# castorini/howl

Hardware: AMD Instinct MI355X
Metric: utterances/sec/node (res8 end-to-end training step, 1s@16kHz, 40-mel) (higher is better)
Workload: dtype f32; 1 GPU; res8 training step (frontend+fwd+xent+bwd+AdamW), 512 x 1 s utterances per GPU, 12 labels -- BASELINE configs[2] per-GPU share: res8 GSC-12, 512 x 1 s per GPU (4096 over 8); global_batch=512, samples_per_utterance=16000, labels=12, parallelism=single, frontend=eval

## Files before the change

howl_amd/csrc/howl_common.hip.h:

```cpp
#pragma once
#include <hip/hip_runtime.h>
#include <math.h>
#include <stdint.h>
#include <stdio.h>

typedef float f32x4 __attribute__((ext_vector_type(4)));
typedef __attribute__((address_space(3))) float lds_f32;

#if defined(HIPEMU)
#define HOWL_OPAQUE_V(x) ((void)(x))
#else
#define HOWL_OPAQUE_V(x) asm volatile("" : "+v"(x))
#endif
#define HOWL_OPAQUE_LDS(p) HOWL_OPAQUE_V(p)
#if defined(HIPEMU)
#define HOWL_SCHED_PIN() ((void)0)
#else
#define HOWL_SCHED_PIN() __builtin_amdgcn_sched_barrier(0)
#endif

#define HOWL_OK 0
#define HOWL_E_ARG (-1)
#define HOWL_E_LAUNCH (-2)
#define HOWL_E_WORKSPACE (-3)

void howl_set_error(const char* fmt, ...);
int howl_num_cus();
bool howl_prof_begin(const char* tag, hipStream_t stream, size_t* slot, double work);
void howl_prof_end(size_t slot, hipStream_t stream);

struct HowlSideLane {
    hipStream_t stream;
    hipEvent_t fork_ev, join_ev;
};
HowlSideLane* howl_side_lane();
bool howl_raise_lds(const void* kernel, size_t lds, size_t* granted, const char* what);
bool howl_take_pending_error();
inline void howl_lane_fork(HowlSideLane* l, hipStream_t main) {
    hipEventRecord(l->fork_ev, main);
    hipStreamWaitEvent(l->stream, l->fork_ev, 0);
}
inline void howl_lane_join(HowlSideLane* l, hipStream_t main) {
    hipEventRecord(l->join_ev, l->stream);
    hipStreamWaitEvent(main, l->join_ev, 0);
}

struct HowlProfScope {
    size_t slot = 0;
    bool on;
    hipStream_t stream;
    HowlProfScope(const char* tag, hipStream_t s, double work = 0.0) : stream(s) { on = howl_prof_begin(tag, s, &slot, work); }
    ~HowlProfScope() {
        if (on) howl_prof_end(slot, stream);
    }
};

struct HowlAdamWCoef {
    float lr, b1, b2, eps, wd, bc1, bc2_sqrt, gscale;
};
inline HowlAdamWCoef howl_adamw_coef(float lr, float beta1, float beta2, float eps, float weight_decay, int step, float grad_scale) {
    const double bc1 = 1.0 - pow((double)beta1, (double)step);
    const double bc2 = 1.0 - pow((double)beta2, (double)step);
    return HowlAdamWCoef{lr, beta1, beta2, eps, weight_decay, (float)bc1, (float)sqrt(bc2), grad_scale};
}
__device__ __forceinline__ void howl_adamw_element(float* __restrict__ p, float* __restrict__ m, float* __restrict__ v, size_t i, float g,
                                                   const HowlAdamWCoef& c) {
#pragma clang fp contract(off)
    const float gi = g * c.gscale;
    float pi = p[i] * (1.0f - c.lr * c.wd);
    const float mi = m[i] + (gi - m[i]) * (1.0f - c.b1);
    const float vi = c.b2 * v[i] + (1.0f - c.b2) * gi * gi;
    const float denom = sqrtf(vi) / c.bc2_sqrt + c.eps;
    pi -= (c.lr / c.bc1) * (mi / denom);
    p[i] = pi;
    m[i] = mi;
    v[i] = vi;
}

#define HOWL_REQUIRE(cond, ...)                 \
    do {                                        \
        if (!(cond)) {                          \
            howl_set_error(__VA_ARGS__);        \
            return HOWL_E_ARG;                  \
        }                                       \
    } while (0)

#define HOWL_CHECK_LAUNCH(name)                                                     \
    do {                                                                            \
        hipError_t e_ = hipGetLastError();                                          \
        if (howl_take_pending_error()) return HOWL_E_LAUNCH;   \
        if (e_ != hipSuccess) {                                                     \
            howl_set_error("%s: launch failed: %s", name, hipGetErrorString(e_));   \
            return HOWL_E_LAUNCH;                                                   \
        }                                                                           \
    } while (0)

__device__ __forceinline__ void wave_lds_sync() {
    __builtin_amdgcn_fence(__ATOMIC_RELEASE, "wavefront");
    __builtin_amdgcn_wave_barrier();
    __builtin_amdgcn_fence(__ATOMIC_ACQUIRE, "wavefront");
}

__device__ __forceinline__ float wave_sum(float v) {
    for (int m = 32; m >= 1; m >>= 1) v += __shfl_xor(v, m);
    return v;
}
__device__ __forceinline__ float wave_sum_rows(float v) {
    v += __int_as_float(__builtin_amdgcn_update_dpp(0, __float_as_int(v), 0xB1, 0xf, 0xf, true));
    v += __int_as_float(__builtin_amdgcn_update_dpp(0, __float_as_int(v), 0x4E, 0xf, 0xf, true));
    v += __int_as_float(__builtin_amdgcn_update_dpp(0, __float_as_int(v), 0x141, 0xf, 0xf, true));
    v += __int_as_float(__builtin_amdgcn_update_dpp(0, __float_as_int(v), 0x140, 0xf, 0xf, true));
    v += __shfl_xor(v, 16);
    v += __shfl_xor(v, 32);
    return v;
}
__device__ __forceinline__ double wave_sum_d(double v) {
    for (int m = 32; m >= 1; m >>= 1) v += __shfl_xor(v, m);
    return v;
}
```

howl_amd/csrc/res8.hip:

```cpp
#include "howl_common.hip.h"
#include "../../include/howl_hip.h"

namespace {

struct HowlPtrs6 {
    float* p[6];
};
constexpr int MAX_WINDOWS = 64;
struct HowlWinRows {
    int lo[MAX_WINDOWS], hi[MAX_WINDOWS];
};
struct HowlBnBuffers {
    float* running_mean;
    float* running_var;
    long long* num_batches;
};
struct BnFold {
    const float* part;
    int nparts;
    double count;
    float* stats_out;
    HowlBnBuffers bn;
};


constexpr int NMAP = 45;
constexpr int CP = 48;
constexpr int PW = 10;
constexpr int WP = 12;
constexpr int CONV_THREADS = 768;
constexpr int KFULL = 11;
constexpr int KSTEPS = 9 * KFULL + 3;
constexpr int MAX_H = 27;
constexpr int MAX_ROW_STRIPS = 1024;
constexpr float BN_EPS = 1e-5f;
constexpr float BN_MOMENTUM = 0.1f;

__host__ __device__ inline int chan_stride(int H, bool own_rows = false) {
    int cs = (H + (own_rows ? 2 : 1)) * WP;
    int pad = (17 - (cs % 32) + 32) % 32;
    return cs + pad;
}
__host__ __device__ inline int tile_floats(int H, bool own_rows = false) { return CP * chan_stride(H, own_rows) + 32; }
constexpr int WPW = 13;
constexpr int WNCOL = 16 * 26;
constexpr int WTAPS = 9 * NMAP;
__host__ __device__ inline int wgrad_rounds(int H) { return (H + 3) / 4; }

constexpr int PACK_ELEMS = 3 * KSTEPS * 64;
__device__ __forceinline__ void pack_weights_one(const HowlPtrs6& w, float* __restrict__ wp_fwd, float* __restrict__ wp_bwd,
                                                 int layer, int mode, int idx) {
    const int lane = idx & 63;
    const int ks = (idx >> 6) % KSTEPS;
    const int nt = idx / (64 * KSTEPS);
    int kk, tap;
    if (ks < 9 * KFULL) {
        const int c0 = ks / 9;
        tap = ks - 9 * c0;
        kk = 4 * c0 + (lane >> 4);
    } else {
        tap = 4 * (ks - 9 * KFULL) + (lane >> 4);
        kk = 4 * KFULL;
    }
    const int n = 16 * nt + (lane & 15);
    float v = 0.0f;
    if (kk < NMAP && n < NMAP && tap < 9) {
        const float* wl = w.p[layer];
        v = (mode == 0) ? wl[(n * NMAP + kk) * 9 + tap] : wl[(kk * NMAP + n) * 9 + (8 - tap)];
    }
    float* dst = (mode == 0 ? wp_fwd : wp_bwd) + (size_t)layer * (3 * KSTEPS * 64);
    dst[idx] = v;
}

__device__ __forceinline__ void zero_lds(float* p, int n, int tid, int nthreads) {
    const int n4 = n >> 2;
    for (int i = tid; i < n4; i += nthreads) reinterpret_cast<float4*>(p)[i] = make_float4(0.0f, 0.0f, 0.0f, 0.0f);
    for (int i = 4 * n4 + tid; i < n; i += nthreads) p[i] = 0.0f;
}

__host__ __device__ inline int part_stride(int nparts) { return (nparts + 3) & ~3; }
__device__ __forceinline__ double fold_part_column(const float* __restrict__ part, int nps, int nparts, int column, int lane) {
    const int slice = lane & 7;
    const float* src = part + (size_t)column * nps;
    double acc = 0.0;
    for (int r0 = 4 * slice; r0 < nparts; r0 += 8 * 32) {
        float4 v[8];
#pragma unroll
        for (int j = 0; j < 8; ++j) {
            const int r = r0 + 32 * j;
            v[j] = *reinterpret_cast<const float4*>(src + (r < nps ? r : 0));
        }
#pragma unroll
        for (int j = 0; j < 8; ++j) {
            const int r = r0 + 32 * j;
            acc += (r + 0 < nparts) ? (double)v[j].x : 0.0;
            acc += (r + 1 < nparts) ? (double)v[j].y : 0.0;
            acc += (r + 2 < nparts) ? (double)v[j].z : 0.0;
            acc += (r + 3 < nparts) ? (double)v[j].w : 0.0;
        }
    }
    acc += __shfl_xor(acc, 1);
    acc += __shfl_xor(acc, 2);
    acc += __shfl_xor(acc, 4);
    return acc;
}

template <int NTW>
struct KCursor {
    const lds_f32* ap[NTW];
    const lds_f32* bp;
    float a[NTW], b;
};

template <int NTW>
__device__ __forceinline__ void k_prime(KCursor<NTW>& k) {
#pragma unroll
    for (int i = 0; i < NTW; ++i) k.a[i] = k.ap[i][0];
    k.b = k.bp[0];
}

template <int NTW, int TS>
__device__ __forceinline__ void k_begin(KCursor<NTW>& k, f32x4 (&acc)[NTW], const lds_f32* tile, const lds_f32* wl,
                                        int CS, int P, int t0, int lane) {
    constexpr int ts = TS;
#pragma unroll
    for (int i = 0; i < NTW; ++i) {
        int m = 16 * (t0 + ts * i) + (lane & 15);
        m = m < P ? m : P - 1;
        const int h = m / PW;
        k.ap[i] = tile + (lane >> 4) * CS + h * WP + (m - h * PW);
        HOWL_OPAQUE_LDS(k.ap[i]);
        acc[i] = {0.0f, 0.0f, 0.0f, 0.0f};
    }
    k.bp = wl + lane;
    HOWL_OPAQUE_LDS(k.bp);
}

template <int NTW>
__device__ __forceinline__ void k_run(KCursor<NTW>& k, f32x4 (&acc)[NTW], int CS, int groups) {
#pragma unroll 2
    for (int g = 0; g < groups; ++g) {
#pragma unroll
        for (int tap = 0; tap < 9; ++tap) {
            float na[NTW], nb;
            if (tap < 8) {
                const int off = ((tap + 1) / 3) * WP + ((tap + 1) % 3);
#pragma unroll
                for (int i = 0; i < NTW; ++i) na[i] = k.ap[i][off];
                nb = k.bp[(tap + 1) * 64];
            } else {
                k.bp += 9 * 64;
#pragma unroll
                for (int i = 0; i < NTW; ++i) k.ap[i] += 4 * CS;
#pragma unroll
// ... 1428 lines not shown
                const unsigned bc = (4u * idx[u] + 2u * h) / (unsigned)P;
                const unsigned bb = bc / NMAP;
                cc[u][h] = bc - bb * NMAP;
                if (dx == nullptr) gb[h] = dpool[bb * CP + cc[u][h]] * invP;
            }
            g[u] = dx != nullptr ? reinterpret_cast<const float4*>(dx)[idx[u]] : make_float4(gb[0], gb[0], gb[1], gb[1]);
            sv[u] = reinterpret_cast<const float4*>(s)[idx[u]];
            kk[u] = dskip != nullptr ? reinterpret_cast<const float4*>(dskip)[idx[u]] : make_float4(0.0f, 0.0f, 0.0f, 0.0f);
        }
#pragma unroll
        for (int u = 0; u < 2; ++u) {
            float2 dsa, dza, dsb, dzb;
            finish(make_float2(g[u].x, g[u].y), make_float2(sv[u].x, sv[u].y), make_float2(kk[u].x, kk[u].y), cc[u][0], dsa, dza);
            finish(make_float2(g[u].z, g[u].w), make_float2(sv[u].z, sv[u].w), make_float2(kk[u].z, kk[u].w), cc[u][1], dsb, dzb);
            if (ok[u]) {
                if (ds_out != nullptr) reinterpret_cast<float4*>(ds_out)[idx[u]] = make_float4(dsa.x, dsa.y, dsb.x, dsb.y);
                reinterpret_cast<float4*>(dz_out)[idx[u]] = make_float4(dza.x, dza.y, dzb.x, dzb.y);
            }
        }
    }
    if ((n2 & 1u) && blockIdx.x == 0 && tid == 0) {
        const unsigned i = n2 - 1;
        const unsigned bc = (2u * i) / (unsigned)P;
        const unsigned bb = bc / NMAP, c = bc - bb * NMAP;
        float2 g;
        if (dx != nullptr) {
            g = reinterpret_cast<const float2*>(dx)[i];
        } else {
            const float v = dpool[bb * CP + c] * invP;
            g = make_float2(v, v);
        }
        const float2 sv = reinterpret_cast<const float2*>(s)[i];
        const float2 kk = dskip != nullptr ? reinterpret_cast<const float2*>(dskip)[i] : make_float2(0.0f, 0.0f);
        float2 ds, dz;
        finish(g, sv, kk, c, ds, dz);
        if (ds_out != nullptr) reinterpret_cast<float2*>(ds_out)[i] = ds;
        reinterpret_cast<float2*>(dz_out)[i] = dz;
    }
}


template <bool EXACT = false>
__device__ __forceinline__ void load_feat_tile(float* tin, const float* feat, long sb, long st, long sm, int b, int T,
                                               int M, int tid, int nthreads, int t_lo = 0, int t_hi = 0) {
    const int pitch = M + 4;
    const int n = (T + 2) * pitch;
    for (int i0 = tid; i0 < n; i0 += 8 * nthreads) {
        float v[8];
#pragma unroll
        for (int j = 0; j < 8; ++j) {
            const int i = i0 + j * nthreads;
            const int t = i / pitch - 1, m = i % pitch - 1;
            const bool ok = i < n && (EXACT ? t >= t_lo && t < t_hi : t >= 0 && t < T) && m >= 0 && m < M;
            v[j] = feat[b * sb + (ok ? t * st + m * sm : 0)];
        }
#pragma unroll
        for (int j = 0; j < 8; ++j) {
            const int i = i0 + j * nthreads;
            const int t = i / pitch - 1, m = i % pitch - 1;
            const bool ok = (EXACT ? t >= t_lo && t < t_hi : t >= 0 && t < T) && m >= 0 && m < M;
            if (i < n) tin[i] = ok ? v[j] : 0.0f;
        }
    }
}

constexpr int C0M_THREADS = 512;

template <int NS = 1, bool EXACT = false>
__global__ __launch_bounds__(C0M_THREADS) void conv0_fwd_mfma_kernel(const float* __restrict__ feat, long sb, long st,
                                                                    long sm, const float* __restrict__ w0,
                                                                    float* __restrict__ s0, unsigned short* __restrict__ mask0,
                                                                    int B, int T, int M, int H, int nconv, HowlPtrs6 cw,
                                                                    float* __restrict__ wp_fwd, float* __restrict__ wp_bwd,
                                                                    int nwin, int win_step, int win_last, int slices) {
    if ((int)blockIdx.x >= nconv) {
        const int e = ((int)blockIdx.x - nconv) * C0M_THREADS + (int)threadIdx.x;
        if (e < 2 * 6 * PACK_ELEMS) pack_weights_one(cw, wp_fwd, wp_bwd, (e / PACK_ELEMS) % 6, e / (6 * PACK_ELEMS), e % PACK_ELEMS);
        return;
    }
    HIP_DYNAMIC_SHARED(float, lds)
    float* tin = lds;
    const int tid = threadIdx.x, lane = tid & 63, wave = tid >> 6;
    const int pitch = M + 4;
    const int P = H * PW;
    const int g = lane >> 4, n = lane & 15;
    float bw[3][3];
#pragma unroll
    for (int ks = 0; ks < 3; ++ks)
#pragma unroll
        for (int nt = 0; nt < 3; ++nt) {
            const int tap = 4 * ks + g, c = 16 * nt + n;
            bw[ks][nt] = (tap < 9 && c < NMAP) ? w0[c * 9 + tap] : 0.0f;
        }
    int aoff[3];
#pragma unroll
    for (int ks = 0; ks < 3; ++ks) {
        const int tap = min(4 * ks + g, 8);
        aoff[ks] = (tap / 3) * pitch + tap % 3 + (n & 7) + (n >> 3) * 3 * pitch;
    }
    for (int i = tid; i < 3 * pitch + 16; i += C0M_THREADS) tin[(T + 2) * pitch + i] = 0.0f;
    for (int item = blockIdx.x; item < B * slices; item += nconv) {
        const int b = item / slices, sl = item - b * slices;
        const int ph0 = (sl * H) / slices, ph1 = ((sl + 1) * H) / slices;
        __syncthreads();
        const int clip = b / nwin, wi = b - clip * nwin;
        const int t0 = EXACT ? wi * win_step : min(wi * win_step, win_last);
        load_feat_tile<EXACT>(tin, feat + (long)clip * sb + (long)t0 * st, 0, st, sm, 0, T, M, tid, C0M_THREADS, -t0, win_last - t0);
        __syncthreads();
        constexpr int NJ = 5 * NS;
        for (int u = wave; u < NJ * ((ph1 - ph0 + 1) / 2); u += C0M_THREADS / 64) {
            const int pp = u / NJ, j8 = u - NJ * pp;
            const float* rowp = tin + 3 * (ph0 + 2 * pp) * pitch + 8 * j8;
            {
                f32x4 acc[3][3];
#pragma unroll
                for (int tl = 0; tl < 3; ++tl)
#pragma unroll
                    for (int nt = 0; nt < 3; ++nt) acc[tl][nt] = {0.0f, 0.0f, 0.0f, 0.0f};
#pragma unroll
                for (int tl = 0; tl < 3; ++tl)
#pragma unroll
                    for (int ks = 0; ks < 3; ++ks) {
                        const float a = rowp[aoff[ks] + tl * pitch];
#pragma unroll
                        for (int nt = 0; nt < 3; ++nt)
                            acc[tl][nt] = __builtin_amdgcn_mfma_f32_16x16x4f32(a, bw[ks][nt], acc[tl][nt], 0, 0, 0);
                    }
                const int pw = 2 * j8 + (g & 1), ph = ph0 + 2 * pp + (g >> 1);
#pragma unroll
                for (int nt = 0; nt < 3; ++nt) {
                    float sum = 0.0f;
                    unsigned bits = 0;
#pragma unroll
                    for (int tl = 0; tl < 3; ++tl)
#pragma unroll
                        for (int r = 0; r < 4; ++r) {
                            const int rb = max(__float_as_int(acc[tl][nt][r]), 0);
                            sum += __int_as_float(rb);
                            bits |= min((unsigned)rb, 1u) << (4 * tl + r);
                        }
                    const int c = 16 * nt + n;
                    if (ph < ph1 && c < NMAP) {
                        const int strip = NS > 1 ? pw / PW : 0;
                        const size_t o = (((size_t)b * NS + strip) * NMAP + c) * P + (size_t)ph * PW + (pw - strip * PW);
                        s0[o] = sum * (1.0f / 12.0f);
                        if (mask0 != nullptr) mask0[o] = (unsigned short)bits;
                    }
                }
            }
        }
    }
}

constexpr int C0G_WAVES = 15, C0G_THREADS = 64 * C0G_WAVES, C0G_CPW = NMAP / C0G_WAVES;
static_assert(C0G_CPW * C0G_WAVES == NMAP, "channels split evenly over the waves");

__device__ __forceinline__ void load_patch(float (&x)[5][6], const float* tin, int pitch, int ph, int pw) {
    const float* base = tin + 3 * ph * pitch + 4 * pw;
#pragma unroll
    for (int r = 0; r < 5; ++r) {
        const float4 a = *reinterpret_cast<const float4*>(base + r * pitch);
        const float2 c = *reinterpret_cast<const float2*>(base + r * pitch + 4);
        x[r][0] = a.x, x[r][1] = a.y, x[r][2] = a.z, x[r][3] = a.w, x[r][4] = c.x, x[r][5] = c.y;
    }
}

template <int NS = 1, bool EXACT = false>
__global__ __launch_bounds__(C0G_THREADS) void conv0_wgrad_valu_kernel(const float* __restrict__ feat, long sb, long st, long sm,
                                                                      const unsigned short* __restrict__ mask0,
                                                                      const float* __restrict__ ga, const float* __restrict__ gb,
                                                                      float* __restrict__ part, int B, int T, int M, int H,
                                                                      int slices, StripGeom sg, int t_total) {
    HIP_DYNAMIC_SHARED(float, lds)
    float* tin = lds;
    const int tid = threadIdx.x, lane = tid & 63;
    const int wave = __builtin_amdgcn_readfirstlane(tid >> 6);
    const int pitch = M + 4;
    const int P = H * PW;
    float acc[C0G_CPW][9];
#pragma unroll
    for (int j = 0; j < C0G_CPW; ++j)
#pragma unroll
        for (int t = 0; t < 9; ++t) acc[j][t] = 0.0f;
    const int nrs = EXACT ? sg.nr : 1;
    for (int item = blockIdx.x; item < B * nrs * NS * slices; item += gridDim.x) {
        const int vb = item / slices, sl = item - vb * slices;
        const int vq = NS > 1 ? vb / NS : vb, strip = NS > 1 ? vb - vq * NS : 0;
        const int b = EXACT ? vq / nrs : vq, rs = EXACT ? vq - b * nrs : 0;
        const int Pv = (EXACT && rs == nrs - 1) ? sg.hv_last * PW : P;
        const int cell0 = (sl * Pv) / slices, cell1 = ((sl + 1) * Pv) / slices;
        __syncthreads();
        if constexpr (EXACT)
            load_feat_tile<true>(tin, feat + (long)rs * T * st, sb, st, sm, b, T, M, tid, C0G_THREADS, -rs * T, t_total - rs * T);
        else
            load_feat_tile(tin, feat, sb, st, sm, b, T, M, tid, C0G_THREADS);
        __syncthreads();
        const float* gab = ga + ((size_t)vb * NMAP + C0G_CPW * wave) * P;
        const float* gbb = gb != nullptr ? gb + ((size_t)vb * NMAP + C0G_CPW * wave) * P : nullptr;
        const unsigned short* mb = mask0 + ((size_t)vb * NMAP + C0G_CPW * wave) * P;
        for (int cb = cell0; cb < cell1; cb += 64) {
            const int cell = cb + lane;
            const bool valid = cell < cell1;
            const unsigned cc = (unsigned)(valid ? cell : cell1 - 1);
            float gv[C0G_CPW];
            unsigned mv[C0G_CPW];
#pragma unroll
            for (int j = 0; j < C0G_CPW; ++j) {
                const unsigned o = (unsigned)(j * P) + cc;
                gv[j] = gab[o] + (gbb != nullptr ? gbb[o] : 0.0f);
                mv[j] = mb[o];
            }
            const int ph = (int)cc / PW, pw = (int)cc - ph * PW;
            float x[5][6];
            load_patch(x, tin, pitch, ph, pw + strip * PW);
#pragma unroll
            for (int j = 0; j < C0G_CPW; ++j) {
                const int gbits = valid ? __float_as_int(gv[j] * (1.0f / 12.0f)) : 0;
#pragma unroll
                for (int tl = 0; tl < 3; ++tl)
#pragma unroll
                    for (int fl = 0; fl < 4; ++fl) {
                        const int k = 4 * tl + fl;
                        const int sel = ((int)(mv[j] << (31 - k))) >> 31;
                        const float dy = __int_as_float(sel & gbits);
#pragma unroll
                        for (int tap = 0; tap < 9; ++tap) acc[j][tap] = fmaf(dy, x[tl + tap / 3][fl + tap % 3], acc[j][tap]);
                    }
            }
        }
    }
#pragma unroll
    for (int j = 0; j < C0G_CPW; ++j)
#pragma unroll
        for (int t = 0; t < 9; ++t) {
            const float v = wave_sum_rows(acc[j][t]);
            if (lane == 0) part[(size_t)blockIdx.x * NMAP * 9 + (C0G_CPW * wave + j) * 9 + t] = v;
        }
}

constexpr int HEAD_XC = 64;
constexpr int HEAD_THREADS = 768, HEAD_PARTS = 16;
__global__ __launch_bounds__(HEAD_THREADS) void head_fwd_kernel(const float* __restrict__ s6, const float* __restrict__ stats,
                                                       const float* __restrict__ wout, const float* __restrict__ bout,
                                                       float* __restrict__ pooled, float* __restrict__ logits, int B,
                                                       int P, int C, const long long* __restrict__ labels,
                                                       float* __restrict__ nll, float* __restrict__ dlogits,
                                                       float* __restrict__ dpool, float inv_batch,
                                                       const float* __restrict__ pool, int npg, int npg_used, BnFold fold,
                                                       int ns ) {
    __shared__ float lp[CP];
    __shared__ float ll[HEAD_XC], dl[HEAD_XC], lse_s;
    __shared__ float lst[2 * CP];
    __shared__ float lw[HEAD_XC * NMAP];
    __shared__ float lparts[HEAD_PARTS][CP];
    const int tid = threadIdx.x, lane = tid & 63, wave = tid >> 6;
    const bool w_in_lds = C <= HEAD_XC;
    if (w_in_lds)
        for (int i = tid; i < C * NMAP; i += HEAD_THREADS) lw[i] = wout[i];
    if (fold.part != nullptr) {
        const int c8 = lane >> 3;
        for (int w0 = wave; w0 < CP / 4; w0 += HEAD_THREADS / 64) {
            const int c = 4 * w0 + (c8 & 3);
            const double sm = fold_part_column(fold.part, part_stride(fold.nparts), fold.nparts, (c8 < 4 ? 0 : CP) + c, lane);
            const double q = __shfl_xor(sm, 32);
            if (c8 < 4 && (lane & 7) == 0) {
                const double mean = sm / fold.count;
                double var = q / fold.count - mean * mean;
                var = var < 0.0 ? 0.0 : var;
                const float fm = (c < NMAP) ? (float)mean : 0.0f;
                const float fr = (c < NMAP) ? (float)(1.0 / sqrt(var + (double)BN_EPS)) : 0.0f;
                lst[c] = fm;
                lst[CP + c] = fr;
                if (blockIdx.x == 0) {
                    fold.stats_out[c] = fm;
                    fold.stats_out[CP + c] = fr;
                    if (c < NMAP && fold.bn.running_mean != nullptr) {
                        const double unbiased = fold.count > 1.0 ? var * fold.count / (fold.count - 1.0) : var;
                        fold.bn.running_mean[c] = (1.0f - BN_MOMENTUM) * fold.bn.running_mean[c] + BN_MOMENTUM * (float)mean;
                        fold.bn.running_var[c] = (1.0f - BN_MOMENTUM) * fold.bn.running_var[c] + BN_MOMENTUM * (float)unbiased;
                    }
                    if (c == 0 && fold.bn.num_batches != nullptr) fold.bn.num_batches[0] += 1;
                }
            }
        }
    } else if (tid < 2 * CP) {
        lst[tid] = stats[tid];
    }
    __syncthreads();
    for (int b = blockIdx.x; b < B; b += gridDim.x) {
        __syncthreads();
        if (pool != nullptr) {
            const int nparts = ns * npg_used;
            const int pc = tid % CP, pk = tid / CP;
            float acc = 0.0f;
            for (int k0 = 0; k0 < nparts; k0 += HEAD_PARTS) {
                const int k = k0 + pk;
                if (k < nparts) {
                    const int sgi = k / npg_used, g = k - sgi * npg_used;
                    lparts[pk][pc] = pool[(((size_t)b * ns + sgi) * npg + g) * CP + pc];
                }
                __syncthreads();
                if (tid < CP) {
                    const int n = nparts - k0 < HEAD_PARTS ? nparts - k0 : HEAD_PARTS;
                    for (int j = 0; j < n; ++j) acc += lparts[j][tid];
                }
                __syncthreads();
            }
            if (tid < CP) {
                const float v = tid < NMAP ? (acc / (float)P - lst[tid]) * lst[CP + tid] : 0.0f;
                lp[tid] = v;
                pooled[(size_t)b * CP + tid] = v;
            }
        } else if (wave < 4)
        for (int c0 = wave; c0 < CP; c0 += 12) {
            float a8[3][8];
#pragma unroll
            for (int u = 0; u < 3; ++u) {
                const int c = c0 + 4 * u < NMAP ? c0 + 4 * u : NMAP - 1;
                const float* src = s6 + ((size_t)b * NMAP + c) * P;
#pragma unroll
                for (int j = 0; j < 8; ++j) a8[u][j] = src[min(lane + 64 * j, P - 1)];
            }
#pragma unroll
            for (int u = 0; u < 3; ++u) {
                const int c = c0 + 4 * u;
#pragma unroll
                for (int j = 0; j < 8; ++j) a8[u][j] = (lane + 64 * j < P) ? fabsf(a8[u][j]) : 0.0f;
                float acc = ((a8[u][0] + a8[u][1]) + (a8[u][2] + a8[u][3])) + ((a8[u][4] + a8[u][5]) + (a8[u][6] + a8[u][7]));
                acc = wave_sum(acc);
                const float v = c < NMAP ? (acc / (float)P - lst[c]) * lst[CP + c] : 0.0f;
                if (lane == 0 && c < CP) {
                    lp[c] = v;
                    pooled[(size_t)b * CP + c] = v;
                }
            }
        }
        __syncthreads();
        for (int k = tid; k < C; k += HEAD_THREADS) {
            float acc = bout[k];
            if (w_in_lds)
                for (int c = 0; c < NMAP; ++c) acc = fmaf(lw[k * NMAP + c], lp[c], acc);
            else
                for (int c = 0; c < NMAP; ++c) acc = fmaf(wout[k * NMAP + c], lp[c], acc);
            logits[(size_t)b * C + k] = acc;
            if (labels != nullptr) ll[k] = acc;
        }
        if (labels == nullptr) continue;
        __syncthreads();
        const int y = (int)labels[b];
        if (tid == 0) {
            float mx = ll[0];
            for (int k = 1; k < C; ++k) mx = fmaxf(mx, ll[k]);
            float se = 0.0f;
            for (int k = 0; k < C; ++k) se += expf(ll[k] - mx);
            const float lse = mx + logf(se);
            lse_s = lse;
            nll[b] = lse - ll[y];
        }
        __syncthreads();
        if (tid < C) {
            const float d = (expf(ll[tid] - lse_s) - (tid == y ? 1.0f : 0.0f)) * inv_batch;
            dl[tid] = d;
            dlogits[(size_t)b * C + tid] = d;
        }
        __syncthreads();
        if (tid < CP) {
            float acc = 0.0f;
            if (tid < NMAP)
                for (int k = 0; k < C; ++k) acc = fmaf(dl[k], lw[k * NMAP + tid], acc);
            dpool[(size_t)b * CP + tid] = acc;
        }
    }
}

__global__ __launch_bounds__(256) void head_fwd_windows_kernel(const float* __restrict__ s6, const float* __restrict__ stats,
                                                               const float* __restrict__ wout, const float* __restrict__ bout,
                                                               float* __restrict__ logits, int B, int nwin, int Hw,
                                                               HowlWinRows rows, float inv_count, int C, int ns) {
    __shared__ float lp[CP];
    const int tid = threadIdx.x, lane = tid & 63, wave = tid >> 6;
    const int Pw = Hw * PW;
    for (int b = blockIdx.x; b < B; b += gridDim.x) {
        __syncthreads();
        for (int c = wave; c < CP; c += 4) {
            float acc = 0.0f;
            if (c < NMAP) {
                for (int w = 0; w < nwin * ns; ++w) {
                    const float* src = s6 + ((size_t)(b * nwin * ns + w) * NMAP + c) * Pw;
                    for (int i = rows.lo[w / ns] * PW + lane; i < rows.hi[w / ns] * PW; i += 64) acc += fabsf(src[i]);
// ... 143 lines not shown
    if ((threadIdx.x & 63) == 0) red[threadIdx.x >> 6] = acc;
    __syncthreads();
    if (threadIdx.x == 0) {
        double tot = 0.0;
        for (int w = 0; w < 16; ++w) tot += red[w];
        loss[0] = (float)(tot / (double)B);
    }
}

__global__ void adamw_kernel(float* __restrict__ p, const float* __restrict__ g, float* __restrict__ m,
                             float* __restrict__ v, size_t n, HowlAdamWCoef c) {
    for (size_t i = (size_t)blockIdx.x * blockDim.x + threadIdx.x; i < n; i += (size_t)gridDim.x * blockDim.x)
        howl_adamw_element(p, m, v, i, g[i], c);
}

}

namespace {

size_t conv0_tile_floats(int T, int M) { return (size_t)(T + 2) * (M + 4) + 3 * (M + 4) + 16; }
size_t conv_lds_bytes(int H, bool own_rows) {
    return (size_t)(3 * KSTEPS * 64 + tile_floats(H, own_rows) + 4 * CP + 12 * 2 * 16) * sizeof(float);
}
size_t wgrad_lds_bytes(int H) { return (size_t)(tile_floats_z(H) + tile_floats_x(H) + 6 * CP) * sizeof(float); }

struct Ws {
    float* wp_fwd;
    float* wp_bwd;
    float* part;
    float* part2;
    float* stats;
    float* m12;
    float* dpool;
    float* pool;
    float* bufa;
    float* bufb;
    float* dz;
    float* dz2;
    float* dsa;
    float* dsb;
    float* wpart;
    float* c0part;
};

size_t ws_layout(Ws* w, char* base, int B, int H, int G, int cus, size_t* fwd_eval_bytes) {
    size_t off = 0;
    auto take = [&](size_t floats) {
        float* p = base ? reinterpret_cast<float*>(base + off) : nullptr;
        off += ((floats * sizeof(float) + 255) / 256) * 256;
        return p;
    };
    const size_t act = (size_t)B * NMAP * H * PW;
    w->wp_fwd = take((size_t)6 * 3 * KSTEPS * 64);
    w->wp_bwd = take((size_t)6 * 3 * KSTEPS * 64);
    const int max_parts = G > cus ? G : cus;
    w->part = take((size_t)part_stride(max_parts) * 2 * CP);
    w->part2 = take((size_t)part_stride(max_parts) * 2 * CP);
    w->stats = take((size_t)6 * 2 * CP);
    w->m12 = take(2 * CP);
    w->dpool = take((size_t)B * CP);
    w->pool = take((size_t)B * 16 * CP);
    *fwd_eval_bytes = off;
    w->bufa = take(act);
    w->bufb = take(act);
    w->dz = take(act);
    w->dz2 = take(act);
    w->dsa = take(act);
    w->dsb = take(act);
    w->wpart = take((size_t)6 * G * CP * WNCOL);
    w->c0part = take((size_t)max_parts * NMAP * 9);
    return off;
}

int mel_strips(int M) { return M == 40 ? 1 : (M == 80 ? 2 : 0); }
int even_grid(int g, int strips) { return strips > 1 ? ((g & ~1) > 2 ? (g & ~1) : 2) : g; }
int launch_blocks(int nblk, int per_group) { return 8 * per_group * ((nblk + 7) / 8); }
int conv_slices(int nblk, int H, int budget) {
    const int ntiles = (H * PW + 15) / 16;
    for (int sl = 4; sl > 1; sl >>= 1)
        if (nblk * sl <= budget && 4 * sl <= ntiles) return sl;
    return 1;
}
void pair_slices(int nblk, int H, int cus, int* sd, int* sw) {
    const int ntiles = (H * PW + 15) / 16;
    const int opts[3][2] = {{4, 2}, {2, 2}, {2, 1}};
    *sd = *sw = 1;
    for (const auto& o : opts)
        if (nblk * (o[0] + o[1]) <= cus && 4 * o[0] <= ntiles) {
            *sd = o[0];
            *sw = o[1];
            return;
        }
}
int conv0_slices(int B, int cus) {
    const int sl = cus / (B > 0 ? B : 1);
    return sl < 1 ? 1 : (sl > 8 ? 8 : sl);
}
bool env_off(const char* name) {
    const char* e = getenv(name);
    return e != nullptr && e[0] == '0';
}

constexpr int WIN_H = MAX_H, WIN_MARGIN = 7, WIN_STEP = WIN_H - 2 * WIN_MARGIN;
int long_windows(int H) { return H <= WIN_H ? 1 : (H - WIN_H + WIN_STEP - 1) / WIN_STEP + 1; }

struct Res8Plan {
    int B, T, M, ns, nr, Hs, hv_last, Bv, halo;
    StripGeom sg;
    int P, Pt;
    bool slicing, merged, fused;
    int G, SL;
    size_t lds_conv;
    int Bw, Tw, S0, G0, c0_nwin, c0_step, c0_last;
    bool c0_exact;
    size_t lds_conv0;
    int Gh, SD, SW, ew_grid;
    bool fold_in_pair;
    size_t wpart_stride, lds_wgrad, lds_pair;
    int S0w, G0w;
    size_t lds_conv0w;
    size_t saved_floats, train_bytes, eval_bytes;
    size_t long_map_bytes, long_bytes;
    Ws ws;
};

void plan_launches(Res8Plan& p, bool slice_conv0, char* ws_base) {
    const int cus = howl_num_cus(), H = p.Hs;
    p.P = H * PW;
    p.Pt = (p.T / 3) * PW * p.ns;
    p.saved_floats = (size_t)p.Bv * NMAP * p.P;
    p.slicing = !env_off("HOWL_RES8_SLICES");
    p.merged = !env_off("HOWL_RES8_BWD_PAIR");
    p.fused = p.halo != 0 || !env_off("HOWL_RES8_BWD_FUSED");

    p.G = even_grid(p.Bv < cus ? p.Bv : cus, p.ns);
    p.SL = p.halo == 0 && p.slicing ? conv_slices(p.G, H, cus) : 1;
    p.lds_conv = conv_lds_bytes(H, p.halo == 2);
    p.S0 = slice_conv0 && p.slicing ? conv0_slices(p.Bw, cus) : 1;
    p.G0 = p.Bw * p.S0 < 2 * cus ? p.Bw * p.S0 : 2 * cus;
    p.lds_conv0 = conv0_tile_floats(p.Tw, p.M) * sizeof(float);

    const int half = cus / 2 > 0 ? cus / 2 : 1;
    p.Gh = even_grid(p.Bv < half ? p.Bv : half, p.ns);
    p.SD = p.SW = 1;
    if (p.halo == 0 && p.slicing) pair_slices(p.Gh, H, cus, &p.SD, &p.SW);
    p.fold_in_pair = p.Gh * p.SD >= 64;
    p.wpart_stride = (size_t)p.Gh * CP * WNCOL;
    p.lds_wgrad = wgrad_lds_bytes(H);
    p.lds_pair = p.lds_conv > p.lds_wgrad ? p.lds_conv : p.lds_wgrad;
    const size_t quads = (p.saved_floats / 4 + BRB_THREADS - 1) / BRB_THREADS;
    p.ew_grid = quads < 1 ? 1 : (quads > (size_t)(2 * cus) ? 2 * cus : (int)quads);
    p.S0w = p.slicing ? conv0_slices(p.Bv, cus) : 1;
    p.G0w = p.Bv * p.S0w < cus ? p.Bv * p.S0w : cus;
    p.lds_conv0w = ((size_t)(p.Tw + 2) * (p.M + 4) + 16) * sizeof(float);

    p.train_bytes = ws_layout(&p.ws, ws_base, p.Bv, H, p.G, cus, &p.eval_bytes);
}

Res8Plan res8_plan(int B, int T, int M, void* ws = nullptr) {
    Res8Plan p{};
    const int H = T / 3;
    p.B = B, p.T = T, p.M = M;
    p.ns = mel_strips(M) > 0 ? mel_strips(M) : 1;
    p.nr = H <= MAX_H ? 1 : (H + MAX_H - 1) / MAX_H;
    p.Hs = (H + p.nr - 1) / p.nr;
    p.hv_last = H - (p.nr - 1) * p.Hs;
    p.Bv = B * p.nr * p.ns;
    p.halo = p.nr > 1 ? 2 : (p.ns > 1 ? 1 : 0);
    p.sg = StripGeom{p.nr, p.ns, p.hv_last};
    p.c0_exact = p.halo == 2;
    p.Bw = B * p.nr;
    p.Tw = p.c0_exact ? 3 * p.Hs : T;
    p.c0_nwin = p.c0_exact ? p.nr : 1;
    p.c0_step = p.c0_exact ? 3 * p.Hs : 0;
    p.c0_last = p.c0_exact ? T : 0;
    plan_launches(p, true, static_cast<char*>(ws));
    return p;
}

Res8Plan res8_long_plan(int B, int T, int M, void* ws = nullptr) {
    Res8Plan p{};
    const int H = T / 3, nw = long_windows(H);
    p.B = B, p.T = T, p.M = M;
    p.ns = mel_strips(M) > 0 ? mel_strips(M) : 1;
    p.nr = 1, p.Hs = p.hv_last = WIN_H;
    p.Bv = B * nw * p.ns;
    p.halo = p.ns > 1 ? 1 : 0;
    p.sg = StripGeom{1, 1, 0};
    p.Bw = B * nw;
    p.Tw = 3 * WIN_H + T % 3;
    p.c0_nwin = nw, p.c0_step = 3 * WIN_STEP, p.c0_last = 3 * (H - WIN_H);
    static_assert((6 * 2 * CP * sizeof(float)) % 256 == 0, "statistics block keeps the 256-byte alignment");
    p.long_map_bytes = ((size_t)p.Bv * NMAP * WIN_H * PW * sizeof(float) + 255) / 256 * 256;
    const size_t front = 3 * p.long_map_bytes + 6 * 2 * CP * sizeof(float) + 256;
    plan_launches(p, false, ws ? static_cast<char*>(ws) + front : nullptr);
    p.long_bytes = front + p.train_bytes;
    return p;
}

int check_workspace(const char* who, size_t have, size_t need) {
    if (have >= need) return HOWL_OK;
    howl_set_error("%s: workspace %zu < %zu bytes", who, have, need);
    return HOWL_E_WORKSPACE;
}
template <class T>
HowlPtrs6 ptrs6(T* const (&a)[6]) {
    HowlPtrs6 r;
    for (int i = 0; i < 6; ++i) r.p[i] = const_cast<float*>(a[i]);
    return r;
}
StageCfg plain_tile(const float* t) { return StageCfg{t, nullptr, nullptr, nullptr, nullptr, 0.0f, false, false, false}; }

template <auto Kernel>
void raise_lds_limit(size_t lds) {
    static thread_local size_t granted[16] = {};
    howl_raise_lds(reinterpret_cast<const void*>(Kernel), lds, granted, "res8 kernel");
}
template <int HALO>
StripGeom geom_arg(const Res8Plan& p) { return HALO == 2 ? p.sg : StripGeom{1, 1, 0}; }

struct Conv3x3Launch {
    StageCfg in;
    const float* in_stats = nullptr;
    const float* wp = nullptr;
    const float* res = nullptr;
    float* out = nullptr;
    const float* xs = nullptr;
    const float* xs_stats = nullptr;
    float* part = nullptr;
    float* pool = nullptr;
    BnFold fold{};
    BwdFold bfold{};
    WFold wf{nullptr, 0, nullptr};
};
template <int MODE, int SLICES, int HALO>
void launch_conv3x3_inst(const Res8Plan& p, hipStream_t stream, const Conv3x3Launch& a) {
    const int nblk = MODE == 0 ? p.G : p.Gh;
    raise_lds_limit<conv3x3_mfma_kernel<MODE, SLICES, HALO>>(p.lds_conv);
    hipLaunchKernelGGL((conv3x3_mfma_kernel<MODE, SLICES, HALO>), dim3(launch_blocks(nblk, SLICES)), dim3(CONV_THREADS), p.lds_conv,
                       stream, a.in, a.in_stats, a.wp, a.res, a.out, a.xs, a.xs_stats, a.part, a.pool, p.Bv, p.Hs, nblk, a.fold,
                       a.bfold, a.wf, geom_arg<HALO>(p));
}
template <int MODE>
void launch_conv3x3(const Res8Plan& p, hipStream_t stream, const Conv3x3Launch& a) {
    const int slices = MODE == 0 ? p.SL : p.SD;
    if (p.halo == 2)
        launch_conv3x3_inst<MODE, 1, 2>(p, stream, a);
    else if (p.halo == 1)
        launch_conv3x3_inst<MODE, 1, 1>(p, stream, a);
    else if (slices == 4)
        launch_conv3x3_inst<MODE, 4, 0>(p, stream, a);
    else if (slices == 2)
        launch_conv3x3_inst<MODE, 2, 0>(p, stream, a);
    else
        launch_conv3x3_inst<MODE, 1, 0>(p, stream, a);
}

struct BwdLayerLaunch {
    StageCfg zc;
    BwdFold bfold;
    const float* wp;
    float* dx;
    const float* xs;
    const float* xs_stats;
    float* spart;
    const float* s_prev;
    const float* in_stats;
    float* wpart;
    WFold wf;
};
template <int SD, int SW, int HALO>
void launch_pair_inst(const Res8Plan& p, hipStream_t stream, const BwdLayerLaunch& a) {
    raise_lds_limit<bwd_pair_kernel<SD, SW, HALO>>(p.lds_pair);
    hipLaunchKernelGGL((bwd_pair_kernel<SD, SW, HALO>), dim3(launch_blocks(p.Gh, SD + SW)), dim3(CONV_THREADS), p.lds_pair, stream, a.zc,
                       a.bfold, a.wp, a.dx, a.xs, a.xs_stats, a.spart, a.s_prev, a.in_stats, a.wpart, p.Bv, p.Hs, p.Gh, a.wf,
                       geom_arg<HALO>(p));
}
void launch_pair(const Res8Plan& p, hipStream_t stream, const BwdLayerLaunch& a) {
    if (p.halo == 2)
        launch_pair_inst<1, 1, 2>(p, stream, a);
    else if (p.halo == 1)
        launch_pair_inst<1, 1, 1>(p, stream, a);
    else if (p.SD == 4 && p.SW == 2)
        launch_pair_inst<4, 2, 0>(p, stream, a);
    else if (p.SD == 2 && p.SW == 2)
        launch_pair_inst<2, 2, 0>(p, stream, a);
    else if (p.SD == 2 && p.SW == 1)
        launch_pair_inst<2, 1, 0>(p, stream, a);
    else
        launch_pair_inst<1, 1, 0>(p, stream, a);
}
template <int SW, int HALO>
void launch_wgrad_inst(const Res8Plan& p, hipStream_t stream, const BwdLayerLaunch& a) {
    StageCfg zw = a.zc;
    zw.ds = nullptr;
    raise_lds_limit<wgrad_mfma_kernel<SW, HALO>>(p.lds_wgrad);
    hipLaunchKernelGGL((wgrad_mfma_kernel<SW, HALO>), dim3(launch_blocks(p.Gh, SW)), dim3(CONV_THREADS), p.lds_wgrad, stream,
                       WStage{zw, a.s_prev, false}, a.in_stats, a.bfold, a.wpart, p.Bv, p.Hs, p.Gh, geom_arg<HALO>(p));
}
void launch_wgrad(const Res8Plan& p, hipStream_t stream, const BwdLayerLaunch& a) {
    if (p.halo == 2)
        launch_wgrad_inst<1, 2>(p, stream, a);
    else if (p.halo == 1)
        launch_wgrad_inst<1, 1>(p, stream, a);
    else if (p.SW == 2)
        launch_wgrad_inst<2, 0>(p, stream, a);
    else
// ... 329 lines not shown
```

Before: 472,000 utterances/sec.

## Restructure conv0 weight-gradient kernel with packed FMA, two-item tiles and prefetch

The conv0 weight-gradient VALU kernel now uses 12 waves of 4 channels each instead of 15 waves of 3, and pairs channels so that v_pk_fma_f32 updates two accumulators per instruction, with v_bfe_i32 used to extract mask bits. Each block now processes two work items per iteration, loading both feature tiles into doubled LDS and running one combined cell stream over them. The next 64 cells' gradient and mask operands are software-prefetched while the current ones are computed. The aims are to halve FMA instruction count, cut loop and sync overhead per item, and hide global-load latency. In exchange it doubles LDS use, leaves the last wave mostly idle on a single channel, and adds inline asm and register pressure.

```diff
diff --git a/howl_amd/csrc/howl_common.hip.h b/howl_amd/csrc/howl_common.hip.h
--- a/howl_amd/csrc/howl_common.hip.h
+++ b/howl_amd/csrc/howl_common.hip.h
@@ -5,6 +5,7 @@
 #include <stdio.h>
 
 typedef float f32x4 __attribute__((ext_vector_type(4)));
+typedef float f32x2 __attribute__((ext_vector_type(2)));
 typedef __attribute__((address_space(3))) float lds_f32;
 
 #if defined(HIPEMU)
@@ -18,6 +19,29 @@
 #else
 #define HOWL_SCHED_PIN() __builtin_amdgcn_sched_barrier(0)
 #endif
+template <int K>
+__device__ __forceinline__ int howl_bit_select(unsigned m) {
+#if defined(HIPEMU)
+    return ((int)(m << (31 - K))) >> 31;
+#else
+    int r;
+    asm("v_bfe_i32 %0, %1, %2, 1" : "=v"(r) : "v"(m), "n"(K));
+    return r;
+#endif
+}
+template <int HALF>
+__device__ __forceinline__ void howl_pk_fma_bcast(f32x2& acc, f32x2 a, f32x2 x) {
+#if defined(HIPEMU)
+    const float xv = HALF ? x.y : x.x;
+    acc.x = fmaf(a.x, xv, acc.x);
+    acc.y = fmaf(a.y, xv, acc.y);
+#else
+    if (HALF)
+        asm("v_pk_fma_f32 %0, %1, %2, %0 op_sel:[0,1,0] op_sel_hi:[1,1,1]" : "+v"(acc) : "v"(a), "v"(x));
+    else
+        asm("v_pk_fma_f32 %0, %1, %2, %0 op_sel:[0,0,0] op_sel_hi:[1,0,1]" : "+v"(acc) : "v"(a), "v"(x));
+#endif
+}
 
 #define HOWL_OK 0
 #define HOWL_E_ARG (-1)
diff --git a/howl_amd/csrc/res8.hip b/howl_amd/csrc/res8.hip
--- a/howl_amd/csrc/res8.hip
+++ b/howl_amd/csrc/res8.hip
@@ -1,5 +1,6 @@
 #include "howl_common.hip.h"
 #include "../../include/howl_hip.h"
+#include <utility>
 
 namespace {
 
@@ -1734,17 +1735,70 @@
     }
 }
 
-constexpr int C0G_WAVES = 15, C0G_THREADS = 64 * C0G_WAVES, C0G_CPW = NMAP / C0G_WAVES;
-static_assert(C0G_CPW * C0G_WAVES == NMAP, "channels split evenly over the waves");
-
-__device__ __forceinline__ void load_patch(float (&x)[5][6], const float* tin, int pitch, int ph, int pw) {
+constexpr int C0G_WAVES = 12, C0G_THREADS = 64 * C0G_WAVES, C0G_CPW = 4;
+static_assert(C0G_CPW * C0G_WAVES >= NMAP && C0G_CPW * (C0G_WAVES - 1) + 1 == NMAP, "the last wave holds channel 44 alone");
+__host__ __device__ inline int conv0w_tile_floats(int T, int M) { return (T + 2) * (M + 4) + 16; }
+
+__device__ __forceinline__ void load_patch(f32x2 (&x)[5][3], const float* tin, int pitch, int ph, int pw) {
     const float* base = tin + 3 * ph * pitch + 4 * pw;
 #pragma unroll
     for (int r = 0; r < 5; ++r) {
-        const float4 a = *reinterpret_cast<const float4*>(base + r * pitch);
-        const float2 c = *reinterpret_cast<const float2*>(base + r * pitch + 4);
-        x[r][0] = a.x, x[r][1] = a.y, x[r][2] = a.z, x[r][3] = a.w, x[r][4] = c.x, x[r][5] = c.y;
-    }
+        const f32x4 a = *reinterpret_cast<const f32x4*>(base + r * pitch);
+        x[r][0] = f32x2{a.x, a.y}, x[r][1] = f32x2{a.z, a.w};
+        x[r][2] = *reinterpret_cast<const f32x2*>(base + r * pitch + 4);
+    }
+}
+
+struct C0gOps {
+    float g[C0G_CPW], g2[C0G_CPW];
+    unsigned m[C0G_CPW];
+};
+struct C0gItem {
+    int vb, b, rs, strip, cell0, n;
+};
+template <int NS, bool EXACT>
+__device__ __forceinline__ C0gItem c0g_item(int item, int slices, int nrs, int P, const StripGeom& sg) {
+    C0gItem it;
+    const int vb = item / slices, sl = item - vb * slices;
+    const int vq = NS > 1 ? vb / NS : vb;
+    it.vb = vb;
+    it.strip = NS > 1 ? vb - vq * NS : 0;
+    it.b = EXACT ? vq / nrs : vq;
+    it.rs = EXACT ? vq - it.b * nrs : 0;
+    const int Pv = (EXACT && it.rs == nrs - 1) ? sg.hv_last * PW : P;
+    it.cell0 = (sl * Pv) / slices;
+    it.n = ((sl + 1) * Pv) / slices - it.cell0;
+    return it;
+}
+__device__ __forceinline__ void c0g_request(C0gOps& o, const float* gab, const float* gbb, const unsigned short* mb, unsigned off,
+                                            unsigned PJ) {
+#pragma unroll
+    for (int j = 0; j < C0G_CPW; ++j) {
+        const unsigned e = off + (unsigned)j * PJ;
+        o.g[j] = gab[e];
+        o.g2[j] = gbb != nullptr ? gbb[e] : 0.0f;
+        o.m[j] = mb[e];
+    }
+}
+template <int K>
+__device__ __forceinline__ void c0g_position(f32x2 (&acc)[9], const f32x2 (&x)[5][3], unsigned m0, unsigned m1, int g0, int g1) {
+    constexpr int tl = K / 4, fl = K % 4;
+    f32x2 dy;
+    dy.x = __int_as_float(howl_bit_select<K>(m0) & g0);
+    dy.y = __int_as_float(howl_bit_select<K>(m1) & g1);
+#pragma unroll
+    for (int tap = 0; tap < 9; ++tap) {
+        const int col = fl + tap % 3;
+        if (col & 1)
+            howl_pk_fma_bcast<1>(acc[tap], dy, x[tl + tap / 3][col >> 1]);
+        else
+            howl_pk_fma_bcast<0>(acc[tap], dy, x[tl + tap / 3][col >> 1]);
+    }
+}
+template <int... K>
+__device__ __forceinline__ void c0g_pair(f32x2 (&acc)[9], const f32x2 (&x)[5][3], unsigned m0, unsigned m1, int g0, int g1,
+                                         std::integer_sequence<int, K...>) {
+    (c0g_position<K>(acc, x, m0, m1, g0, g1), ...);
 }
 
 template <int NS = 1, bool EXACT = false>
@@ -1754,69 +1808,81 @@
                                                                       float* __restrict__ part, int B, int T, int M, int H,
                                                                       int slices, StripGeom sg, int t_total) {
     HIP_DYNAMIC_SHARED(float, lds)
-    float* tin = lds;
     const int tid = threadIdx.x, lane = tid & 63;
     const int wave = __builtin_amdgcn_readfirstlane(tid >> 6);
     const int pitch = M + 4;
     const int P = H * PW;
-    float acc[C0G_CPW][9];
-#pragma unroll
-    for (int j = 0; j < C0G_CPW; ++j)
-#pragma unroll
-        for (int t = 0; t < 9; ++t) acc[j][t] = 0.0f;
+    const int tile = conv0w_tile_floats(T, M);
+    const int c0 = C0G_CPW * wave;
+    const bool full = c0 + C0G_CPW <= NMAP;
+    const unsigned PJ = full ? (unsigned)P : 0u;
+    f32x2 acc[2][9];
+#pragma unroll
+    for (int p = 0; p < 2; ++p)
+#pragma unroll
+        for (int t = 0; t < 9; ++t) acc[p][t] = f32x2{0.0f, 0.0f};
     const int nrs = EXACT ? sg.nr : 1;
-    for (int item = blockIdx.x; item < B * nrs * NS * slices; item += gridDim.x) {
-        const int vb = item / slices, sl = item - vb * slices;
-        const int vq = NS > 1 ? vb / NS : vb, strip = NS > 1 ? vb - vq * NS : 0;
-        const int b = EXACT ? vq / nrs : vq, rs = EXACT ? vq - b * nrs : 0;
-        const int Pv = (EXACT && rs == nrs - 1) ? sg.hv_last * PW : P;
-        const int cell0 = (sl * Pv) / slices, cell1 = ((sl + 1) * Pv) / slices;
+    const int nitems = B * nrs * NS * slices;
+    const int gstride = (int)gridDim.x;
+    for (int i0 = blockIdx.x; i0 < nitems; i0 += 2 * gstride) {
+        const bool two = i0 + gstride < nitems;
+        const C0gItem ia = c0g_item<NS, EXACT>(i0, slices, nrs, P, sg);
+        const C0gItem ib = c0g_item<NS, EXACT>(two ? i0 + gstride : i0, slices, nrs, P, sg);
+        const int n0 = ia.n, n1 = two ? ib.n : 0;
+        const int nq0 = two ? (n0 + 63) & ~63 : n0, ntot = nq0 + n1;
+        const unsigned dcell = (unsigned)(ib.vb - ia.vb) * (unsigned)(NMAP * P) + (unsigned)ib.cell0;
+        const float* gab = ga + ((size_t)ia.vb * NMAP + c0) * P;
+        const float* gbb = gb != nullptr ? gb + ((size_t)ia.vb * NMAP + c0) * P : nullptr;
+        const unsigned short* mb = mask0 + ((size_t)ia.vb * NMAP + c0) * P;
+        auto cell_offset = [&](int q) {
+            if (q < nq0 || !two) return (unsigned)(ia.cell0 + (q < n0 ? q : n0 - 1));
+            q -= nq0;
+            return dcell + (unsigned)(q < n1 ? q : n1 - 1);
+        };
+        C0gOps ops0, ops1;
+        c0g_request(ops0, gab, gbb, mb, cell_offset(lane), PJ);
         __syncthreads();
-        if constexpr (EXACT)
-            load_feat_tile<true>(tin, feat + (long)rs * T * st, sb, st, sm, b, T, M, tid, C0G_THREADS, -rs * T, t_total - rs * T);
-        else
-            load_feat_tile(tin, feat, sb, st, sm, b, T, M, tid, C0G_THREADS);
+        if constexpr (EXACT) {
+            load_feat_tile<true>(lds, feat + (long)ia.rs * T * st, sb, st, sm, ia.b, T, M, tid, C0G_THREADS, -ia.rs * T, t_total - ia.rs * T);
+            if (two)
+                load_feat_tile<true>(lds + tile, feat + (long)ib.rs * T * st, sb, st, sm, ib.b, T, M, tid, C0G_THREADS, -ib.rs * T,
+                                     t_total - ib.rs * T);
+        } else {
+            load_feat_tile(lds, feat, sb, st, sm, ia.b, T, M, tid, C0G_THREADS);
+            if (two) load_feat_tile(lds + tile, feat, sb, st, sm, ib.b, T, M, tid, C0G_THREADS);
+        }
         __syncthreads();
-        const float* gab = ga + ((size_t)vb * NMAP + C0G_CPW * wave) * P;
-        const float* gbb = gb != nullptr ? gb + ((size_t)vb * NMAP + C0G_CPW * wave) * P : nullptr;
-        const unsigned short* mb = mask0 + ((size_t)vb * NMAP + C0G_CPW * wave) * P;
-        for (int cb = cell0; cb < cell1; cb += 64) {
-            const int cell = cb + lane;
-            const bool valid = cell < cell1;
-            const unsigned cc = (unsigned)(valid ? cell : cell1 - 1);
-            float gv[C0G_CPW];
-            unsigned mv[C0G_CPW];
-#pragma unroll
-            for (int j = 0; j < C0G_CPW; ++j) {
-                const unsigned o = (unsigned)(j * P) + cc;
-                gv[j] = gab[o] + (gbb != nullptr ? gbb[o] : 0.0f);
-                mv[j] = mb[o];
-            }
-            const int ph = (int)cc / PW, pw = (int)cc - ph * PW;
-            float x[5][6];
-            load_patch(x, tin, pitch, ph, pw + strip * PW);
-#pragma unroll
-            for (int j = 0; j < C0G_CPW; ++j) {
-                const int gbits = valid ? __float_as_int(gv[j] * (1.0f / 12.0f)) : 0;
-#pragma unroll
-                for (int tl = 0; tl < 3; ++tl)
-#pragma unroll
-                    for (int fl = 0; fl < 4; ++fl) {
-                        const int k = 4 * tl + fl;
-                        const int sel = ((int)(mv[j] << (31 - k))) >> 31;
-                        const float dy = __int_as_float(sel & gbits);
-#pragma unroll
-                        for (int tap = 0; tap < 9; ++tap) acc[j][tap] = fmaf(dy, x[tl + tap / 3][fl + tap % 3], acc[j][tap]);
-                    }
-            }
-        }
-    }
-#pragma unroll
-    for (int j = 0; j < C0G_CPW; ++j)
+        auto block = [&](const C0gOps& cur, C0gOps& nxt, int qb) __attribute__((always_inline)) {
+            c0g_request(nxt, gab, gbb, mb, cell_offset(qb + 64 + lane), PJ);
+            const int qs = qb + lane;
+            const bool second = two && qs >= nq0;
+            const int r = second ? qs - nq0 : qs, nr = second ? n1 : n0;
+            const bool valid = r < nr;
+            const int cell = (second ? ib.cell0 : ia.cell0) + (valid ? r : nr - 1);
+            const int ph = cell / PW, pw = cell - ph * PW;
+            const int strip = NS > 1 ? (second ? ib.strip : ia.strip) : 0;
+            f32x2 x[5][3];
+            load_patch(x, lds + (second ? tile : 0), pitch, ph, pw + strip * PW);
+            int gbits[C0G_CPW];
+#pragma unroll
+            for (int j = 0; j < C0G_CPW; ++j)
+                gbits[j] = valid && (j == 0 || full) ? __float_as_int((cur.g[j] + cur.g2[j]) * (1.0f / 12.0f)) : 0;
+            c0g_pair(acc[0], x, cur.m[0], cur.m[1], gbits[0], gbits[1], std::make_integer_sequence<int, 12>{});
+            if (full) c0g_pair(acc[1], x, cur.m[2], cur.m[3], gbits[2], gbits[3], std::make_integer_sequence<int, 12>{});
+        };
+        for (int qb = 0; qb < ntot; qb += 128) {
+            block(ops0, ops1, qb);
+            if (qb + 64 < ntot) block(ops1, ops0, qb + 64);
+        }
+    }
+#pragma unroll
+    for (int p = 0; p < 2; ++p)
 #pragma unroll
         for (int t = 0; t < 9; ++t) {
-            const float v = wave_sum_rows(acc[j][t]);
-            if (lane == 0) part[(size_t)blockIdx.x * NMAP * 9 + (C0G_CPW * wave + j) * 9 + t] = v;
+            const float v0 = wave_sum_rows(acc[p][t].x), v1 = wave_sum_rows(acc[p][t].y);
+            const int c = c0 + 2 * p;
+            if (lane == 0 && c < NMAP) part[(size_t)blockIdx.x * NMAP * 9 + c * 9 + t] = v0;
+            if (lane == 0 && c + 1 < NMAP) part[(size_t)blockIdx.x * NMAP * 9 + (c + 1) * 9 + t] = v1;
         }
 }
 
@@ -2266,7 +2332,7 @@
     p.ew_grid = quads < 1 ? 1 : (quads > (size_t)(2 * cus) ? 2 * cus : (int)quads);
     p.S0w = p.slicing ? conv0_slices(p.Bv, cus) : 1;
     p.G0w = p.Bv * p.S0w < cus ? p.Bv * p.S0w : cus;
-    p.lds_conv0w = ((size_t)(p.Tw + 2) * (p.M + 4) + 16) * sizeof(float);
+    p.lds_conv0w = 2 * (size_t)conv0w_tile_floats(p.Tw, p.M) * sizeof(float);
 
     p.train_bytes = ws_layout(&p.ws, ws_base, p.Bv, H, p.G, cus, &p.eval_bytes);
 }
```

Measured after the change: 476,600 utterances/sec, median of 6. Within noise of the previous version (+1.0%).
